# LuoGroup2023/PanTax

Hardware: AMD Instinct MI355X
Metric: PAO wall-time (s) + Mreads/s: packed reads + DB (graphs and their unique-trio index) resident in HBM -> abundance tables; the metric's own GAF -> abundance quantity is value_gaf_to_tables (files -> tables, never `value`) (higher is better)
Workload: dtype int64+f64

## Files before the change

pantax_amd/csrc/common.hpp:

```cpp
#pragma once
#include <hip/hip_runtime.h>
#include <cstdint>
#include <cstdio>
#include <map>
#include <functional>
#include <mutex>
#include <cstring>
#include <atomic>
#include <string>
#include <vector>
#include "../../include/pantax_hip.h"

#ifndef TRIO_LH_PACK
#define TRIO_LH_PACK 0
#endif
namespace ptx {

struct Ctx;
#if TRIO_LH_PACK
using trio_len_t = uint2;
#else
using trio_len_t = uint32_t;
#endif

// ... 274 lines not shown
    DevBuf<uint32_t> d_sp_first_id;
    DevBuf<uint32_t> d_node_base;
    DevBuf<uint64_t> d_bit_off;
    DevBuf<uint32_t> d_node_len;
    DevBuf<uint4> d_node_rec;
    DevBuf<uint64_t> d_path_off;
    DevBuf<uint32_t> d_path_nodes;
    DevBuf<uint32_t> d_hap_species;
    DevBuf<uint64_t> d_hap_off;
    DevBuf<uint8_t> d_all_same;
    std::vector<uint8_t> h_all_same;
    DevBuf<uint2> d_tiles;
    uint64_t n_tiles = 0;
    DevBuf<uint2> d_emit_tile_sp;
    DevBuf<uint64_t> d_node_haps;
    bool nh_built = false, nh_walk_too = false;
    DevBuf<uint32_t> d_tile_rank;
    DevBuf<uint32_t> d_hap_tile_off;
    bool trio_visit_ok = false;
    uint32_t n_vgroups = 0;
    std::vector<uint8_t> h_trio_slow;
    DevBuf<uint32_t> d_trio_slow;
    DevBuf<uint32_t> d_vis_pos;
    DevBuf<uint64_t> d_vis_head;
    DevBuf<uint32_t> d_vis_nbase;
    DevBuf<uint32_t> d_vis_sp;
    DevBuf<uint32_t> d_node_visited;
    bool trio_block_ok = false;
    uint32_t n_blocks = 0;
    uint64_t n_runs = 0;
    DevBuf<uint32_t> d_blk_base;
    DevBuf<uint32_t> d_blk_species;
    DevBuf<uint32_t> d_blk_run_off;
    DevBuf<uint4> d_blk_rec;
    DevBuf<uint4> d_runs;
    bool trio_built = false;
    bool trio_prefetched = false;
    bool trio_keys_built = false;
    bool trio_perm_valid = false;
    uint64_t U = 0;
    bool cov_prepared = false;
    bool cov_count_pending = false;
    bool cov_self_clean = false, cov_arena_clean = false;
    uint64_t cov_arena_sig = 0;
    size_t cov_arena_total = 0;
    hipEvent_t ev_cov_read = nullptr, ev_cov_clean = nullptr;
    bool cov_clean_pending = false;
    bool trio_sizes_known = false;
    uint64_t U_known = 0;
    bool trio_layout_fast = false;
    DevBuf<uint32_t> d_trio_first;
    DevBuf<uint2> d_trio_ent;
#if TRIO_LH_PACK
    DevBuf<uint2> d_trio_len;
#else
    DevBuf<uint32_t> d_trio_len;
    DevBuf<uint16_t> d_trio_hap;
#endif
    DevBuf<uint32_t> d_trio_q;
    DevBuf<uint32_t> d_trio_perm;
    DevBuf<uint64_t> d_hap_trio_off;
    std::vector<uint64_t> h_hap_trio_off;
    std::vector<uint32_t> h_sp_row_order;
    struct NodeChunks { DevBuf<uint32_t> d_chunk_sp, d_sp_off; uint32_t n = 0; };
    NodeChunks node_chunks[2];
    DevBuf<uint4> d_stat_chunks;
    DevBuf<double> d_hs_x;
    DevBuf<uint16_t> d_hs_h;
    DevBuf<uint32_t> d_hs_n;
    uint32_t n_stat_chunks = 0;
    uint64_t n_stat_partials = 0;
    uint32_t stat_lds_haps = 0;
    bool stat_global_rows = false;
    DevBuf<uint32_t> d_sp_chunk_off;
    bool cov_done = false;
    bool cov_stage = false;
    DevBuf<uint8_t> d_cov_arena;
    unsigned long long *d_abort = nullptr;
    DevBuf<unsigned long long> d_bases;
    DevBuf<uint32_t> d_bitmap;
    uint64_t item_sel_layout = 0;
    uint32_t item_sel_n = 0;
    bool item_sel_on = false;
    DevBuf<uint32_t> d_item_sel;
    DevBuf<uint32_t> d_full;
    DevBuf<uint32_t> d_cov;
    DevBuf<unsigned long long> d_trio_bases;
    DevBuf<uint8_t> d_active;
    DevBuf<uint8_t> d_ones;
    DevBuf<unsigned long long> d_counters;
    TrioScratch trio_scratch;
    LadBatch lad;
    DevBuf<uint32_t> d_hap_nnz;
    DevBuf<double> d_hap_mean;
    DevBuf<double> d_hap_part;
    DevBuf<uint8_t> d_arena;
    PinBuf h_arena[2];
    DevBuf<double> d_avg_len, d_sp_abs;
    DevBuf<uint8_t> d_sp_out;
    PinBuf h_sp_out[2];
    hipEvent_t ev_step[2] = {nullptr, nullptr};
    pantax_hip_step_config step_cfg[2];
    int stats_slot = -1;
    int step_enq = 0, step_col = 0, step_inflight = 0;
    hipEvent_t ev_trio_free = nullptr;
    bool trio_free_valid = false;
    bool trio_free_pending = false;
    ~Db() { for (hipEvent_t e : ev_step) if (e) (void)hipEventDestroy(e); if (ev_trio_free) (void)hipEventDestroy(ev_trio_free);
            if (ev_cov_read) (void)hipEventDestroy(ev_cov_read); if (ev_cov_clean) (void)hipEventDestroy(ev_cov_clean); }
    DevBuf<uint32_t> d_scan_tmp, d_sort_table, d_ss_ws;
    DevBuf<uint64_t> d_ka[3], d_kb[3];
    DevBuf<uint64_t> d_row16;
};

struct Reads {
    uint64_t R = 0, T = 0;
    DevBuf<uint32_t> d_step_off, d_node_id, d_pstart, d_pend, d_qlen;
    DevBuf<uint8_t> d_mapq, d_flags;
    DevBuf<uint64_t> d_id_hash;
    bool has_flags = false;
    DevBuf<int32_t> d_species;
    std::vector<int32_t> h_pre_species;
    std::vector<uint32_t> h_pre_qlen;
    uint64_t T_pad = 0;
    DevBuf<uint32_t> d_g_node_id, d_g_group_slot, d_slot_of;
    DevBuf<uint4> d_g_read_rec;
    DevBuf<uint8_t> d_g_step_dup;
    DevBuf<uint32_t> d_long_sum;
    DevBuf<uint32_t> d_long_len0;
    uint32_t n_long = 0;
    DevBuf<uint2> d_g_slot_rec;
    DevBuf<uint2> d_g_qm;
    DevBuf<uint2> d_g_mm;
    DevBuf<uint8_t> d_g_flag;
    uint32_t n_slots = 0;
    DevBuf<uint2> d_g_items;
    uint32_t n_items = 0;
    int item_blk_shift = 0;
    bool g_flags_valid = false;
    bool species_valid = false;
    bool binned = false;
    uint64_t binned_db = 0;
    bool grouped = true;
    uint64_t layout_id = 0;
    uint64_t long_sums_db = 0;
    std::vector<uint32_t> h_item_block;
    uint32_t max_node_id = 0;
};

__host__ __device__ inline int slot_species(int32_t x) { return x >= -1 ? x : -x - 2; }

constexpr uint64_t NODE_REC_MAX_BITS = 1ull << 40;
constexpr uint32_t NODE_REC_MAX_ROWS = 1u << 16;
__host__ __device__ inline uint32_t nr_rows(uint32_t y) { return (y >> 8) & 0xFFFFu; }
__host__ __device__ inline uint32_t nr_filter(uint32_t y) { return y >> 24; }
__host__ __device__ inline uint32_t nr_head(uint32_t y_old, uint32_t rows, uint32_t filter) { return (y_old & 0xFFu) | ((rows & 0xFFFFu) << 8) | (filter << 24); }
__host__ __device__ inline uint32_t nr_pair_bit(uint32_t lo, uint32_t hi) { return 1u << (((lo * 0x9E3779B1u) ^ (hi * 0x85EBCA77u)) >> 29); }
__host__ __device__ inline uint64_t nr_bit_off(const uint4 &r) { return ((uint64_t)(r.y & 0xFFu) << 32) | r.x; }
__host__ __device__ inline uint4 nr_make(uint64_t bit_off, uint32_t len) { return make_uint4((uint32_t)bit_off, (uint32_t)(bit_off >> 32) & 0xFFu, len, 0u); }

template <class T>
int upload(Ctx *ctx, DevBuf<T> &dst, const T *src, size_t n) {
    PTX_HIP(ctx, dst.alloc(n));
    if (n) PTX_HIP(ctx, hipMemcpyAsync(dst.p, src, n * sizeof(T), hipMemcpyHostToDevice, ctx->stream));
    return 0;
}
// ... 137 lines not shown
```

pantax_amd/csrc/cov_device.hpp:

```cpp
#pragma once
#include "common.hpp"
#include "wave.hpp"

namespace ptx {

constexpr int COV_BLOCK = 256;

__device__ __forceinline__ uint32_t bm_peek(const uint32_t *p) {
    return __hip_atomic_load(p, __ATOMIC_RELAXED, __HIP_MEMORY_SCOPE_AGENT);
}
constexpr uint32_t COV_BWIN = 2048;
constexpr int COV_WIN = 2048;
extern __shared__ uint32_t s_cov[];
#define S_WIN(i) s_cov[(i)]
#define S_BM(bmo, i) s_cov[(bmo) + (i)]
#define S_FULL(bmo, i) reinterpret_cast<uint8_t *>(s_cov + (bmo) + COV_BWIN)[(i)]
__host__ __device__ constexpr size_t cov_lds_bytes(int win) { return (size_t)win * 4 + COV_BWIN * 4 + (size_t)win; }
__device__ __forceinline__ void lds_or(uint32_t *__restrict__ bm, uint32_t bmo, uint64_t bw0, uint32_t bwn, uint64_t w, uint32_t m) {
    const uint64_t off = w - bw0;
    if (off < bwn) {
        if ((S_BM(bmo, off) & m) != m) atomicOr(&S_BM(bmo, off), m);
    } else if ((bm_peek(&bm[w]) & m) != m) atomicOr(&bm[w], m);
}
__device__ __forceinline__ void mark_range(uint32_t *__restrict__ bm, uint32_t bmo, uint64_t bw0, uint32_t bwn, uint64_t g0, uint64_t g1) {
    if (g1 <= g0) return;
    uint64_t w0 = g0 >> 5, w1 = (g1 - 1) >> 5;
    uint32_t m0 = 0xFFFFFFFFu << (g0 & 31);
    uint32_t m1 = 0xFFFFFFFFu >> (31 - (uint32_t)((g1 - 1) & 31));
    if (w0 == w1) lds_or(bm, bmo, bw0, bwn, w0, m0 & m1);
    else {
        lds_or(bm, bmo, bw0, bwn, w0, m0);
        for (uint64_t w = w0 + 1; w < w1; ++w) lds_or(bm, bmo, bw0, bwn, w, 0xFFFFFFFFu);
        lds_or(bm, bmo, bw0, bwn, w1, m1);
    }
}
__device__ __forceinline__ void win_or(uint32_t bmo, uint32_t w, uint32_t m) { if ((S_BM(bmo, w) & m) != m) atomicOr(&S_BM(bmo, w), m); }
__device__ __forceinline__ void mark_window(uint32_t bmo, uint32_t r0, uint32_t r1) {
    if (r1 <= r0) return;
    const uint32_t w0 = r0 >> 5, w1 = (r1 - 1) >> 5;
    const uint32_t m0 = 0xFFFFFFFFu << (r0 & 31), m1 = 0xFFFFFFFFu >> (31 - ((r1 - 1) & 31));
    if (w0 == w1) win_or(bmo, w0, m0 & m1);
    else {
        win_or(bmo, w0, m0);
        for (uint32_t w = w0 + 1; w < w1; ++w) win_or(bmo, w, 0xFFFFFFFFu);
        win_or(bmo, w1, m1);
    }
}

constexpr uint32_t STEP_LONG = 0x80u;
constexpr uint32_t STEP_START = 0x40u, STEP_PAD = 0xFFu, STEP_DIST = 0x3Fu;
__device__ __forceinline__ unsigned long long ballot1(bool b) { return __builtin_amdgcn_ballot_w64(b); }
__device__ __forceinline__ bool any1(bool b) { return __builtin_amdgcn_ballot_w64(b) != 0ull; }
__device__ __forceinline__ bool none1(bool b) { return __builtin_amdgcn_ballot_w64(b) == 0ull; }
__device__ __forceinline__ uint32_t slot_in_group(uint32_t group_first_slot, uint32_t code, int lane) {
    const unsigned long long starts = ballot1((code != STEP_PAD) & ((code & STEP_START) != 0u)) & ~1ull;
    const uint32_t below = __builtin_amdgcn_mbcnt_hi((uint32_t)(starts >> 32), __builtin_amdgcn_mbcnt_lo((uint32_t)starts, 0u));
    return group_first_slot + below + (uint32_t)((starts >> lane) & 1ull);
}

__device__ __forceinline__ uint32_t rl_from_memory(uint32_t j, uint32_t b, const uint32_t *__restrict__ node_id, const uint8_t *__restrict__ step_dup,
                                                   uint32_t delta, const uint4 *__restrict__ node_rec, uint32_t len0, uint32_t ps) {
    const uint32_t idj = node_id[b + j];
    if (j == 0 || ((step_dup[b + j] & 1u) && idj == node_id[b])) return len0 - ps;
    return node_rec[idj + delta].z;
}

#ifdef COV_ABLATE
#define ABL(bit) (ablate & (bit))
#else
#define ABL(bit) false
#endif
constexpr int COV_WIN_BACK = 128;
constexpr uint32_t NO_SLOT = 0xFFFFFFFFu;

__device__ __forceinline__ void add_bases(unsigned long long *__restrict__ bases, uint32_t wlo, uint32_t win_n, uint32_t v, uint32_t aln) {
    const uint32_t off = v - wlo;
    if (off < win_n && aln < (1u << 18)) atomicAdd(&S_WIN(off), aln);
    else atomicAdd(&bases[v], (unsigned long long)aln);
}
constexpr uint32_t NO_FULL = 0xFFFFFFFFu;
__device__ __forceinline__ void mark_full_wave(uint32_t *__restrict__ full, uint32_t wlo, uint32_t win_n, uint32_t v) {
    const uint32_t off = v - wlo;
    const bool have = v != NO_FULL;
    if (have && off < win_n) S_FULL(COV_WIN, off) = 1;
    const bool out = have && off >= win_n;
    unsigned long long todo = __ballot(out);
    const uint32_t w = v >> 5, bit = 1u << (v & 31);
    const int lane = threadIdx.x & 63;
    while (todo) {
        const int leader = __builtin_ctzll(todo);
        const uint32_t wl = (uint32_t)__builtin_amdgcn_readlane((int)w, leader);
        const bool mine = out && w == wl;
        const uint32_t orv = wave_reduce(mine ? bit : 0u, [](uint32_t x, uint32_t y) { return x | y; });
        if (lane == leader) atomicOr(&full[wl], orv);
        todo &= ~__ballot(mine);
    }
}

constexpr uint32_t COV_ITEM_GROUPS = 128;
struct __attribute__((packed, aligned(4))) EntPair { uint32_t a, b, c, d; };
constexpr int COV_BLK_SHIFT = 11;

template <int WIN>
__device__ __forceinline__ void mark_full_out_wave(uint32_t *__restrict__ full, bool out, uint32_t v) {
    unsigned long long todo = ballot1(out);
    const uint32_t w = v >> 5, bit = 1u << (v & 31);
    const int lane = threadIdx.x & 63;
    while (todo) {
        const int leader = __builtin_ctzll(todo);
        const uint32_t wl = (uint32_t)__builtin_amdgcn_readlane((int)w, leader);
        const bool mine = out & (w == wl);
        const uint32_t orv = wave_reduce(mine ? bit : 0u, [](uint32_t x, uint32_t y) { return x | y; });
        if (lane == leader) atomicOr(&full[wl], orv);
        todo &= ~ballot1(mine);
    }
}

}
```

pantax_amd/csrc/stage_cov.hip:

```cpp
#include <chrono>
#include <cstdio>
#include <cstdlib>
#include "common.hpp"
#include "primitives.hpp"
#include "wave.hpp"
#include "cov_plan.hpp"
#include "cov_device.hpp"
#pragma clang diagnostic ignored "-Wbitwise-instead-of-logical"

namespace ptx {

template <bool WITH_TRIO, int U, int PASSES, int WIN, bool LONG = false>
__global__ void __launch_bounds__(COV_BLOCK) coverage_fast_kernel(
    const uint2 *__restrict__ items, const uint32_t *__restrict__ group_slot, const uint4 *__restrict__ read_rec, const uint2 *__restrict__ slot_rec,
    const uint32_t *__restrict__ node_id, const uint8_t *__restrict__ step_code, const uint8_t *__restrict__ active,
    const uint4 *__restrict__ node_rec, const uint64_t *__restrict__ bit_off, uint64_t V, unsigned long long *__restrict__ bases,
    uint32_t *__restrict__ bitmap, uint32_t *__restrict__ full, const uint2 *__restrict__ trio_ent, unsigned long long *__restrict__ trio_bases,
    unsigned long long *__restrict__ n_abort, uint32_t ablate, int blk_shift,
    const uint32_t *__restrict__ long_sum = nullptr, const uint32_t *__restrict__ long_len0 = nullptr, uint32_t only_long = 0u,
    uint32_t chunk_groups = 0u, uint32_t total_groups = 0u, uint32_t win_back = 0u, const uint32_t *__restrict__ item_sel = nullptr) {
    constexpr int WAVES = COV_BLOCK / 64;
    const int lane = threadIdx.x & 63, wave = threadIdx.x >> 6;
    uint32_t g0, n_groups;
    if constexpr (LONG) { g0 = blockIdx.x * chunk_groups; n_groups = min(g0 + chunk_groups, total_groups); }
    else { const uint2 item = items[item_sel ? item_sel[blockIdx.x] : blockIdx.x]; g0 = item.x; n_groups = item.y; }
    for (int i = threadIdx.x; i < (int)(cov_lds_bytes(WIN) / 4); i += COV_BLOCK) s_cov[i] = 0;
    uint32_t wlo = 0, win_n = 0, mark_n = 0, bit0_lo = 0, bwn = 0;
    uint64_t bw0 = 0;
#pragma unroll 1
    for (uint32_t g = g0; g < n_groups && win_n == 0; ++g) {
        const uint32_t gs = group_slot[g];
        if (gs == NO_SLOT) continue;
        const uint2 sr0 = slot_rec[gs];
        if ((int)sr0.x < 0 || !active[sr0.x]) continue;
        const uint32_t id0 = node_id[(uint64_t)g * 64], v0 = id0 + sr0.y, in_blk = id0 & ((1u << blk_shift) - 1u);
        const uint32_t back = LONG ? win_back : in_blk + 64u;
        wlo = (v0 > back ? v0 - back : 0u) & ~63u;
        win_n = WIN;
        const uint64_t b_lo = bit_off[wlo], b_hi = bit_off[min((uint64_t)wlo + WIN, V)];
        bw0 = b_lo >> 5;
        bit0_lo = (uint32_t)(bw0 << 5);
        bwn = COV_BWIN;
        mark_n = (b_hi - (bw0 << 5) <= (uint64_t)COV_BWIN * 32) ? (uint32_t)min((uint64_t)WIN, V - wlo) : 0u;
    }
    __builtin_amdgcn_fence(__ATOMIC_RELEASE, "workgroup", "local");
    __builtin_amdgcn_s_barrier();
    __builtin_amdgcn_fence(__ATOMIC_ACQUIRE, "workgroup", "local");
#ifndef COV_NO_PREFETCH
    uint32_t n_code[U], n_id[U], n_gs[U];
    {
        const uint32_t gw0 = g0 + (uint32_t)(wave * U);
#pragma unroll
        for (int u = 0; u < U; ++u) {
            const uint32_t g = gw0 + (uint32_t)u < n_groups ? gw0 + (uint32_t)u : (gw0 < n_groups ? gw0 : g0);
            const uint64_t t = (uint64_t)g * 64 + lane;
            n_code[u] = step_code[t]; n_id[u] = node_id[t]; n_gs[u] = group_slot[g];
        }
    }
#endif
#if !defined(COV_NO_PF2) && !defined(COV_NO_PREFETCH)
    constexpr bool PF2 = !LONG;
#else
    constexpr bool PF2 = false;
#endif
    uint32_t c_code[U], c_id[U], c_gs[U];
    uint4 c_rr[U];
    uint2 c_sr[U];
    bool c_run[U];
#pragma unroll
    for (int u = 0; u < U; ++u) c_run[u] = false;
    if constexpr (PF2) {
        const uint32_t gw0 = g0 + (uint32_t)(wave * U), gw1 = gw0 + (uint32_t)(WAVES * U);
#pragma unroll
        for (int u = 0; u < U; ++u) {
            c_code[u] = n_code[u]; c_id[u] = n_id[u]; c_gs[u] = n_gs[u];
            const uint32_t g = gw1 + (uint32_t)u < n_groups ? gw1 + (uint32_t)u : (gw0 < n_groups ? gw0 : g0);
            const uint64_t t = (uint64_t)g * 64 + lane;
            n_code[u] = step_code[t]; n_id[u] = node_id[t]; n_gs[u] = group_slot[g];
            const bool pad0 = c_code[u] == STEP_PAD;
            const bool run0 = (gw0 + (uint32_t)u < n_groups) & any1(!pad0) & none1(!pad0 & ((c_code[u] & STEP_LONG) != 0u));
            const uint32_t sl = slot_in_group(c_gs[u], c_code[u], lane);
            const uint32_t slot = (pad0 | !run0) ? (c_gs[u] == NO_SLOT ? 0u : c_gs[u]) : sl;
            c_rr[u] = read_rec[slot]; c_sr[u] = slot_rec[slot];
            c_run[u] = run0;
        }
    }
#pragma unroll 1
    for (int pass = 0;; ++pass) {
        const uint32_t gw = g0 + (uint32_t)((pass * WAVES + wave) * U);
        if (gw >= n_groups) break;
        uint32_t code[U], id[U], gs[U];
        bool run[U];
        uint4 rr[U];
        uint2 sr[U];
#ifndef COV_NO_PREFETCH
        if constexpr (PF2) {
            const uint32_t gn = gw + (uint32_t)(WAVES * U), g2 = gn + (uint32_t)(WAVES * U);
            uint32_t m_code[U], m_id[U], m_gs[U];
#pragma unroll
            for (int u = 0; u < U; ++u) {
                run[u] = c_run[u];
                code[u] = c_code[u]; id[u] = c_id[u]; gs[u] = c_gs[u]; rr[u] = c_rr[u]; sr[u] = c_sr[u];
                const uint32_t g = g2 + (uint32_t)u < n_groups ? g2 + (uint32_t)u : gw;
                const uint64_t t = (uint64_t)g * 64 + lane;
                m_code[u] = step_code[t]; m_id[u] = node_id[t]; m_gs[u] = group_slot[g];
                const bool padn = n_code[u] == STEP_PAD;
                const bool runn = (gn + (uint32_t)u < n_groups) & any1(!padn) & none1(!padn & ((n_code[u] & STEP_LONG) != 0u));
                const uint32_t sl = slot_in_group(n_gs[u], n_code[u], lane);
                const uint32_t slot = (padn | !runn) ? (n_gs[u] == NO_SLOT ? 0u : n_gs[u]) : sl;
                c_rr[u] = read_rec[slot]; c_sr[u] = slot_rec[slot];
                c_run[u] = runn;
                c_code[u] = n_code[u]; c_id[u] = n_id[u]; c_gs[u] = n_gs[u];
                n_code[u] = m_code[u]; n_id[u] = m_id[u]; n_gs[u] = m_gs[u];
            }
        } else
        {
            const uint32_t gn = gw + (uint32_t)(WAVES * U);
#pragma unroll
            for (int u = 0; u < U; ++u) {
                run[u] = gw + (uint32_t)u < n_groups;
                code[u] = n_code[u]; id[u] = n_id[u]; gs[u] = n_gs[u];
                const uint32_t g = gn + (uint32_t)u < n_groups ? gn + (uint32_t)u : gw;
                const uint64_t t = (uint64_t)g * 64 + lane;
                n_code[u] = step_code[t]; n_id[u] = node_id[t]; n_gs[u] = group_slot[g];
            }
        }
#else
#pragma unroll
        for (int u = 0; u < U; ++u) {
            const uint32_t g = gw + (uint32_t)u;
            run[u] = g < n_groups;
            const uint64_t t = (uint64_t)(run[u] ? g : gw) * 64 + lane;
            code[u] = step_code[t]; id[u] = node_id[t];
            gs[u] = group_slot[run[u] ? g : gw];
        }
#endif
        bool pad[U];
        uint32_t ll0[U], lsum[U];
#pragma unroll
        for (int u = 0; u < U; ++u) {
            pad[u] = code[u] == STEP_PAD;
            if constexpr (!PF2) {
                const bool has_long = any1(!pad[u] & ((code[u] & STEP_LONG) != 0u));
                run[u] = run[u] & any1(!pad[u]) & (LONG ? (has_long | (only_long == 0u)) : !has_long);
            }
            const uint32_t sl = slot_in_group(gs[u], code[u], lane);
            const uint32_t slot = (pad[u] | !run[u]) ? (gs[u] == NO_SLOT ? 0u : gs[u]) : sl;
            if constexpr (!PF2) { rr[u] = read_rec[slot]; sr[u] = slot_rec[slot]; }
            if constexpr (LONG) { ll0[u] = long_len0[slot]; lsum[u] = long_sum[slot]; }
        }
        uint32_t h_id1[U], h_id2[U], h_codes[U];
        if constexpr (LONG) {
#pragma unroll
            for (int u = 0; u < U; ++u) {
                const uint32_t gu = (uint32_t)__builtin_amdgcn_readfirstlane((int)(gw + (uint32_t)u));
                const uint64_t t0 = (uint64_t)(run[u] && gu != 0u ? gu : 1u) * 64;
                h_id1[u] = node_id[t0 - 1]; h_id2[u] = node_id[t0 - 2];
                h_codes[u] = *reinterpret_cast<const uint32_t *>(step_code + t0 - 4);
            }
        }
        uint4 nr[U];
// ... 48 lines not shown
            dead_read[u] = !single[u] & (rr[u].z > len0[u]);
            live[u] = ok[u] & !dead_read[u] & !(single[u] & (rr[u].w < rr[u].z));
            nh[u] = 0; hx[u] = 0; tlo[u] = 0; thi[u] = 0;
            e0[u] = make_uint2(0u, 0u); e1[u] = e0[u];
            if (WITH_TRIO && !ABL(4u)) {
                hx[u] = hw1;
                tlo[u] = min(v[u], v2); thi[u] = max(v[u], v2);
                nh[u] = (live[u] & (i_[u] >= 2u) & ((nr_filter(hy1) & nr_pair_bit(tlo[u], thi[u])) != 0u)) ? nr_rows(hy1) : 0u;
                const EntPair ep = *reinterpret_cast<const EntPair *>(trio_ent + (nh[u] ? hx[u] : 0u));
                e0[u] = make_uint2(ep.a, ep.b); e1[u] = make_uint2(ep.c, ep.d);
            }
        }
#pragma unroll
        for (int u = 0; u < U; ++u) {
            const uint32_t k = rr[u].y, ps = rr[u].z, pe = rr[u].w, i = i_[u];
            if (any1(ok[u] & dead_read[u] & (i == 0u))) { if (ok[u] & dead_read[u] & (i == 0u)) atomicAdd(n_abort, 1ull); }
            const uint32_t contrib = (live[u] & !single[u]) ? (i == 0u ? nl[u] - ps : nl[u]) : 0u;
            const uint32_t pexcl = wave_incl_scan_dpp(contrib) - contrib;
            uint32_t seen = pexcl - __shfl(pexcl, lane - (LONG ? dist[u] : (int)i));
            if constexpr (LONG) seen = cross[u] ? lsum[u] - ps : seen;
            const uint32_t tgt = pe - ps;
            uint32_t aln = nl[u];
            if (i + 1u == k) aln = ((pe >= ps) & (tgt > seen)) ? tgt - seen : 0u;
            if (i == 0u) aln = single[u] ? tgt : nl[u] - ps;
            const uint32_t sidx = i == 0u ? ps : 0u;
            uint32_t hi = sidx + aln;
            if (hi > nl[u]) hi = nl[u];
            const bool markable = live[u] & (hi > sidx) & !(single[u] & !((ps < pe) & (pe <= nl[u])));
            const uint32_t dupd = code[u] & STEP_DIST;
            bool earlier = dupd != 0u, at_step0 = dupd == i;
            if constexpr (LONG) {
                const bool lc = (code[u] & STEP_LONG) != 0u;
                const uint32_t id_first = cross[u] ? idf[u] : __shfl(id[u], lane - dist[u]);
                earlier = lc ? (code[u] & 1u) != 0u : earlier;
                at_step0 = lc ? id[u] == id_first : at_step0;
            }
            const uint32_t rl = !live[u] ? 0u : !earlier ? aln : (at_step0 ? len0[u] - ps : nl[u]);
            const uint32_t off = v[u] - wlo;
            const bool inw = off < win_n;
            if (live[u] & !earlier & (aln != 0u) && !ABL(2u)) {
                if (inw & (aln < (1u << 18))) atomicAdd(&S_WIN(off), aln);
                else atomicAdd(&bases[v[u]], (unsigned long long)aln);
            }
            const bool whole = markable & (sidx == 0u) & (hi == nl[u]);
            if constexpr (LONG) { if (!ABL(1u) && !ABL(8u)) mark_full_out_wave<WIN>(full, whole & !inw, v[u]); }
            if (markable && !ABL(1u)) {
                if (whole) {
                    if (inw) S_FULL(WIN, off) = 1; else if (!LONG && !ABL(8u)) atomicOr(&full[v[u] >> 5], 1u << (v[u] & 31));
                } else if (off < mark_n) {
                    const uint32_t rel = nr[u].x - bit0_lo;
                    mark_window(WIN, rel + sidx, rel + hi);
                } else if (!ABL(8u)) {
                    const uint64_t bo = nr_bit_off(nr[u]);
                    mark_range(bitmap, WIN, bw0, bwn, bo + sidx, bo + hi);
                }
            }
            if (WITH_TRIO && !ABL(4u)) {
                uint32_t rl1 = wave_shr1(rl), rl2 = wave_shr1(rl1);
                if constexpr (LONG) {
                    const uint32_t idf0 = (uint32_t)__builtin_amdgcn_readfirstlane((int)idf[u]), l0 = (uint32_t)__builtin_amdgcn_readfirstlane((int)len0[u]),
                                   ps0 = (uint32_t)__builtin_amdgcn_readfirstlane((int)ps);
                    const uint32_t c1 = h_codes[u] >> 24, c2 = (h_codes[u] >> 16) & 0xFFu;
                    const uint32_t rlh1 = ((i0_[u] == 1u) | (((c1 & 1u) != 0u) & (h_id1[u] == idf0))) ? l0 - ps0 : nrh1[u].z;
                    const uint32_t rlh2 = ((i0_[u] == 2u) | (((c2 & 1u) != 0u) & (h_id2[u] == idf0))) ? l0 - ps0 : nrh2[u].z;
                    rl2 = lane == 0 ? rlh2 : lane == 1 ? rlh1 : rl2;
                    rl1 = lane == 0 ? rlh1 : rl1;
                }
                constexpr uint32_t NO_ROW = 0xFFFFFFFFu;
                const bool m0 = (nh[u] != 0u) & (e0[u].x == tlo[u]) & (e0[u].y == thi[u]);
                const bool m1 = (nh[u] > 1u) & (e1[u].x == tlo[u]) & (e1[u].y == thi[u]);
                uint32_t row = m0 ? hx[u] : m1 ? hx[u] + 1u : NO_ROW;
                if (any1(!(m0 | m1) & (nh[u] > 2u))) {
                    if (!(m0 | m1) & (nh[u] > 2u))
                        for (uint32_t j = 2; j < nh[u]; ++j) {
                            const uint2 e = trio_ent[hx[u] + j];
                            if (e.x == tlo[u] && e.y == thi[u]) { row = hx[u] + j; break; }
                        }
                }
                const uint32_t sum = rl2 + rl1 + rl;
                if ((row != NO_ROW) & (sum != 0u)) atomicAdd(&trio_bases[row], (unsigned long long)sum);
            }
        }
    }
    __syncthreads();
    if (win_n) {
        for (int i = threadIdx.x; i < WIN; i += COV_BLOCK) {
            const uint32_t c = S_WIN(i);
            if (c) atomicAdd(&bases[wlo + i], (unsigned long long)c);
            const unsigned long long fb = __ballot(S_FULL(WIN, i) != 0);
            if (fb && (lane & 31) == 0 && !ABL(32u)) {
                const uint32_t m = (uint32_t)(fb >> (lane & 32));
                if (m) atomicOr(&full[(wlo + i) >> 5], m);
            }
        }
        if (!ABL(16u))
        for (uint32_t i = threadIdx.x; i < bwn; i += COV_BLOCK) {
            const uint32_t m = S_BM(WIN, i);
            if (m) atomicOr(&bitmap[bw0 + i], m);
        }
    }
}

template <int WS_U, bool EAGER = false>
__global__ void __launch_bounds__(256) walk_sum_kernel(uint64_t T, const uint32_t *__restrict__ group_slot, const uint8_t *__restrict__ step_dup,
                                                       const uint4 *__restrict__ read_rec, const uint2 *__restrict__ slot_rec,
                                                       const uint32_t *__restrict__ node_id, const uint32_t *__restrict__ node_len,
                                                       uint32_t *__restrict__ long_sum, uint32_t *__restrict__ long_len0) {
    const int lane = threadIdx.x & 63;
    const uint64_t stride = (uint64_t)gridDim.x * 256 * WS_U;
    for (uint64_t base = ((uint64_t)blockIdx.x * 256 + (threadIdx.x - lane)) * WS_U; base < T; base += stride) {
        uint32_t code[WS_U], slot[WS_U], id[WS_U], nl[WS_U], gs_e[WS_U], id_e[WS_U];
        uint64_t t[WS_U];
        bool any = false;
#pragma unroll
        for (int u = 0; u < WS_U; ++u) {
            t[u] = base + (uint64_t)u * 64 + lane;
            code[u] = t[u] < T ? step_dup[t[u]] : STEP_PAD;
            if constexpr (EAGER) { gs_e[u] = t[u] < T ? group_slot[t[u] >> 6] : NO_SLOT; id_e[u] = t[u] < T ? node_id[t[u]] : 0u; }
        }
#pragma unroll
        for (int u = 0; u < WS_U; ++u) any = any || (code[u] != STEP_PAD && (code[u] & STEP_LONG));
        if (!__any(any)) continue;
#pragma unroll
        for (int u = 0; u < WS_U; ++u) {
            slot[u] = NO_SLOT; id[u] = 0;
            uint32_t gs;
            if constexpr (EAGER) gs = gs_e[u]; else gs = t[u] < T ? group_slot[t[u] >> 6] : NO_SLOT;
            const uint32_t sl = slot_in_group(gs, code[u], lane);
            if (code[u] != STEP_PAD && (code[u] & STEP_LONG)) { slot[u] = sl; if constexpr (EAGER) id[u] = id_e[u]; else id[u] = node_id[t[u]]; }
        }
        uint2 sr[WS_U];
        uint4 rr[WS_U];
#pragma unroll
        for (int u = 0; u < WS_U; ++u) {
            sr[u] = make_uint2(0xFFFFFFFFu, 0u); rr[u] = make_uint4(0u, 0u, 0u, 0u);
            if (slot[u] != NO_SLOT) { sr[u] = slot_rec[slot[u]]; rr[u] = read_rec[slot[u]]; }
        }
#pragma unroll
        for (int u = 0; u < WS_U; ++u) {
            nl[u] = 0;
            const bool counted = slot[u] != NO_SLOT && (int)sr[u].x >= 0 && (uint32_t)(t[u] - rr[u].x) + 1 < rr[u].y;
            if (counted) nl[u] = node_len[id[u] + sr[u].y];
        }
#pragma unroll
        for (int u = 0; u < WS_U; ++u) {
            if (!__any(slot[u] != NO_SLOT)) continue;
            if (slot[u] != NO_SLOT && (int)sr[u].x >= 0 && (uint32_t)(t[u] - rr[u].x) + 1 < rr[u].y && t[u] == rr[u].x)
                long_len0[slot[u]] = nl[u];
            const uint32_t prev = __shfl_up(slot[u], 1);
            const bool head = lane == 0 || prev != slot[u];
            const unsigned long long heads = __ballot(head);
            const int start = 63 - __builtin_clzll(heads & ((2ull << lane) - 1ull));
            const uint32_t sc = wave_incl_scan_dpp(nl[u]);
            const uint32_t front = __shfl(sc, start > 0 ? start - 1 : 0);
            const uint32_t incl = sc - (start > 0 ? front : 0u);
            const unsigned long long after = heads & ~((2ull << lane) - 1ull);
            const bool tail = after ? (lane + 1 == __builtin_ctzll(after)) : lane == 63;
            if (tail && slot[u] != NO_SLOT && incl) atomicAdd(&long_sum[slot[u]], incl);
        }
    }
}

__global__ void __launch_bounds__(256) popcount_kernel(uint64_t V, const uint64_t *__restrict__ bit_off, const uint32_t *__restrict__ full,
                                                       const uint32_t *__restrict__ bitmap, uint32_t *__restrict__ cov) {
    for (uint64_t v = (uint64_t)blockIdx.x * 256 + threadIdx.x; v < V; v += (uint64_t)gridDim.x * 256) {
        uint64_t g0 = bit_off[v], g1 = bit_off[v + 1];
        uint32_t c = 0;
        if ((full[v >> 5] >> (uint32_t)(v & 31)) & 1u) c = (uint32_t)(g1 - g0);
        else if (g1 > g0) {
            uint64_t w0 = g0 >> 5, w1 = (g1 - 1) >> 5;
            uint32_t m0 = 0xFFFFFFFFu << (g0 & 31);
            uint32_t m1 = 0xFFFFFFFFu >> (31 - (uint32_t)((g1 - 1) & 31));
            if (w0 == w1) c = __popc(bitmap[w0] & m0 & m1);
            else {
                c = __popc(bitmap[w0] & m0);
                for (uint64_t w = w0 + 1; w < w1; ++w) c += __popc(bitmap[w]);
                c += __popc(bitmap[w1] & m1);
            }
        }
        cov[v] = c;
    }
}

// ... 80 lines not shown
            PTX_HIP(ctx, hipStreamSynchronize(ctx->stream));
            if (nz) return fail(ctx, PANTAX_HIP_E_STATE, "coverage_prepare: %llu non-zero words in an arena its last readers should have left clean", nz);
        }
        PTX_HIP(ctx, hipMemsetAsync(db->d_abort, 0, 8, ctx->stream));
    } else {
        KTimer t(ctx, "zero_fill_kernel");
        PTX_TRY(zero_fill(ctx, base, total));
    }
    db->cov_arena_clean = false;
    db->cov_arena_sig = sig;
    if (rd->R && rd->T_pad && rd->n_long && rd->long_sums_db != 0 && rd->long_sums_db == db->uid) {
    } else if (rd->R && rd->T_pad && rd->n_long) {
        PTX_HIP(ctx, hipMemsetAsync(rd->d_long_sum.p, 0, rd->R * sizeof(uint32_t), ctx->stream));
        KTimer t(ctx, "walk_sum_kernel");
        const bool eager = (uint64_t)rd->n_long * 2 > rd->n_slots;
        hipLaunchKernelGGL((eager ? walk_sum_kernel<4, true> : walk_sum_kernel<4, false>), dim3(grid_for(rd->T_pad / 4 + 1, 256, ctx->n_cu * 16)), dim3(256), 0, ctx->stream, rd->T_pad, rd->d_g_group_slot.p,
                           rd->d_g_step_dup.p, rd->d_g_read_rec.p, rd->d_g_slot_rec.p, rd->d_g_node_id.p, db->d_node_len.p, rd->d_long_sum.p,
                           rd->d_long_len0.p);
    }
    PTX_HIP(ctx, hipGetLastError());
    db->cov_prepared = true;
    return 0;
}

int coverage_arena_clean_async(Ctx *ctx, Db *db) {
    if (!db->d_cov_arena.p || !db->cov_arena_total || !ctx->stream2) return 0;
    uint8_t *f_ptr = db->d_cov_arena.p;
    const size_t f_n = db->cov_arena_total;
    if (!db->ev_cov_read) PTX_HIP(ctx, hipEventCreateWithFlags(&db->ev_cov_read, hipEventDisableTiming));
    if (!db->ev_cov_clean) PTX_HIP(ctx, hipEventCreateWithFlags(&db->ev_cov_clean, hipEventDisableTiming));
    PTX_HIP(ctx, hipEventRecord(db->ev_cov_read, ctx->stream));
    PTX_HIP(ctx, hipStreamWaitEvent(ctx->stream2, db->ev_cov_read, 0));
    hipStream_t main_stream = ctx->stream;
    ctx->stream_main = main_stream; ctx->stream = ctx->stream2;
    int rc;
    rc = zero_fill(ctx, f_ptr, f_n);
    const hipError_t e = hipEventRecord(db->ev_cov_clean, ctx->stream2);
    ctx->stream = main_stream; ctx->stream_main = nullptr;
    if (rc != 0) return rc;
    PTX_HIP(ctx, e);
    db->cov_done = false;
    db->cov_arena_clean = true; db->cov_clean_pending = true;
    return 0;
}

struct CovLap {
    Ctx *ctx;
    bool on;
    std::chrono::steady_clock::time_point prev = std::chrono::steady_clock::now();
    void operator()(const char *what) {
        if (!on) return;
        (void)hipStreamSynchronize(ctx->stream);
        const auto now = std::chrono::steady_clock::now();
        std::fprintf(stderr, "[node_coverage]        %-28s %9.3f ms\n", what, std::chrono::duration<double, std::milli>(now - prev).count());
        prev = now;
    }
};

static int active_flags(Ctx *ctx, Db *db, const uint8_t *d_active, const uint8_t **out) {
    if (!d_active) {
        if (db->d_ones.n < db->S) { PTX_HIP(ctx, db->d_ones.alloc(db->S)); PTX_HIP(ctx, hipMemsetAsync(db->d_ones.p, 1, db->S, ctx->stream)); }
        d_active = db->d_ones.p;
    }
    *out = d_active;
    return 0;
}

struct ItemList { uint32_t n; const uint32_t *d; };
static int item_selection(Ctx *ctx, Db *db, const Reads *rd, ItemList *out) {
    *out = {rd->n_items, nullptr};
    if (db->item_sel_layout == rd->layout_id && rd->layout_id != 0) {
        *out = {db->item_sel_n, db->item_sel_on ? db->d_item_sel.p : nullptr};
    } else if (rd->h_item_block.size() == rd->n_items && rd->item_blk_shift > 0 && db->S && !db->h_range_start.empty()) {
        const CovItemSel s = cov_item_select(rd->h_item_block, rd->item_blk_shift, db->h_range_start, db->h_range_end);
        if (s.on && s.n_sel) PTX_TRY(upload(ctx, db->d_item_sel, s.sel.data(), s.sel.size()));
        *out = {s.n_sel, s.on && s.n_sel ? db->d_item_sel.p : nullptr};
        db->item_sel_layout = rd->layout_id; db->item_sel_n = s.n_sel; db->item_sel_on = s.on;
    }
    return 0;
}

struct CovFastTail {
    const uint2 *items; int blk_shift; const uint32_t *long_sum, *long_len0; uint32_t only_long, chunk_groups, total_groups, win_back; const uint32_t *item_sel;
};
template <int U, int PASSES, int WIN, bool LONG>
static void fast_launch_as(Ctx *ctx, Db *db, Reads *rd, const uint8_t *d_act, bool trio, int grid, const CovFastTail &t) {
    if (grid <= 0) return;
    const auto kernel = trio ? coverage_fast_kernel<true, U, PASSES, WIN, LONG> : coverage_fast_kernel<false, U, PASSES, WIN, LONG>;
    hipLaunchKernelGGL(kernel, dim3(grid), dim3(COV_BLOCK), cov_lds_bytes(WIN), ctx->stream, t.items, rd->d_g_group_slot.p, rd->d_g_read_rec.p,
                       rd->d_g_slot_rec.p, rd->d_g_node_id.p, rd->d_g_step_dup.p, d_act, db->d_node_rec.p, db->d_bit_off.p, db->V, db->d_bases.p,
                       db->d_bitmap.p, db->d_full.p, db->d_trio_ent.p, db->d_trio_bases.p, db->d_abort, ctx->cfg.cov_ablate ,
                       t.blk_shift, t.long_sum, t.long_len0, t.only_long, t.chunk_groups, t.total_groups, t.win_back, t.item_sel);
}

static int fast_launch(Ctx *ctx, Db *db, Reads *rd, const uint8_t *d_act, bool trio, const CovFastShape &f, const ItemList &list) {
    const CovFastTail t{rd->d_g_items.p, rd->item_blk_shift, nullptr, nullptr, 0u, 0u, 0u, 0u, list.d};
    const int grid = (int)list.n;
    const auto is = [&](int u, int passes, int win) { return f.u == u && f.passes == passes && f.win == win; };
    if (is(1, 8, 2048)) fast_launch_as<1, 8, 2048, false>(ctx, db, rd, d_act, trio, grid, t);
    else if (is(2, 4, 2048)) fast_launch_as<2, 4, 2048, false>(ctx, db, rd, d_act, trio, grid, t);
    else if (is(2, 8, 2048)) fast_launch_as<2, 8, 2048, false>(ctx, db, rd, d_act, trio, grid, t);
    else if (is(2, 8, 3072)) fast_launch_as<2, 8, 3072, false>(ctx, db, rd, d_act, trio, grid, t);
    else if (is(2, 8, 4096)) fast_launch_as<2, 8, 4096, false>(ctx, db, rd, d_act, trio, grid, t);
    else if (is(2, 4, 3072)) fast_launch_as<2, 4, 3072, false>(ctx, db, rd, d_act, trio, grid, t);
    else if (is(2, 8, 2304)) fast_launch_as<2, 8, 2304, false>(ctx, db, rd, d_act, trio, grid, t);
    else if (is(2, 8, 2560)) fast_launch_as<2, 8, 2560, false>(ctx, db, rd, d_act, trio, grid, t);
    else if (is(2, 4, 2304)) fast_launch_as<2, 4, 2304, false>(ctx, db, rd, d_act, trio, grid, t);
    else if (is(2, 4, 2560)) fast_launch_as<2, 4, 2560, false>(ctx, db, rd, d_act, trio, grid, t);
    else if (is(1, 8, 2304)) fast_launch_as<1, 8, 2304, false>(ctx, db, rd, d_act, trio, grid, t);
    else if (is(4, 4, 2304)) fast_launch_as<4, 4, 2304, false>(ctx, db, rd, d_act, trio, grid, t);
    else if (is(4, 4, 2048)) fast_launch_as<4, 4, 2048, false>(ctx, db, rd, d_act, trio, grid, t);
    else if (is(4, 4, 3072)) fast_launch_as<4, 4, 3072, false>(ctx, db, rd, d_act, trio, grid, t);
    else return fail(ctx, PANTAX_HIP_E_STATE, "coverage_launch: no short-read kernel of shape U = %d, PASSES = %d, WIN = %d", f.u, f.passes, f.win);
    return 0;
}

static int long_launch(Ctx *ctx, Db *db, Reads *rd, const uint8_t *d_act, bool trio, const CovPlan &plan) {
    if (!rd->d_long_sum.p) { PTX_HIP(ctx, rd->d_long_sum.alloc(rd->R)); PTX_HIP(ctx, rd->d_long_len0.alloc(rd->R)); }
    const CovLongShape &l = plan.lng;
    const uint32_t total_groups = (uint32_t)(rd->T_pad / 64);
    const int grid = (int)((total_groups + l.chunk_groups - 1) / l.chunk_groups);
    const CovFastTail t{nullptr, 0, rd->d_long_sum.p, rd->d_long_len0.p, plan.only_long ? 1u : 0u, l.chunk_groups, total_groups, l.win_back, nullptr};
    if (l.u == 1 && l.win == 2048) fast_launch_as<1, 1, 2048, true>(ctx, db, rd, d_act, trio, grid, t);
    else if (l.u == 1 && l.win == 3072) fast_launch_as<1, 1, 3072, true>(ctx, db, rd, d_act, trio, grid, t);
    else if (l.u == 1 && l.win == 4096) fast_launch_as<1, 1, 4096, true>(ctx, db, rd, d_act, trio, grid, t);
    else if (l.u == 2 && l.win == 2048) fast_launch_as<2, 1, 2048, true>(ctx, db, rd, d_act, trio, grid, t);
    else if (l.u == 2 && l.win == 4096) fast_launch_as<2, 1, 4096, true>(ctx, db, rd, d_act, trio, grid, t);
    else if (l.u == 2 && l.win == 3072) fast_launch_as<2, 1, 3072, true>(ctx, db, rd, d_act, trio, grid, t);
    else return fail(ctx, PANTAX_HIP_E_STATE, "coverage_launch: no long-walk kernel of shape U = %d, WIN = %d", l.u, l.win);
    return 0;
}

static int count_launch(Ctx *ctx, Db *db) {
    PTX_HIP(ctx, db->d_cov.alloc(db->V));
    KTimer t(ctx, "popcount_kernel");
    if (long_node_shape(db->L, db->V, ctx->cfg.ncs_prefix_min, ctx->cfg.ncs_no_prefix))
        hipLaunchKernelGGL(popcount_long_kernel, dim3(grid_for((db->V + 63) / 64, 4, ctx->n_cu * 8)), dim3(256), 0, ctx->stream, db->V,
                           db->d_bit_off.p, db->d_full.p, db->d_bitmap.p, db->d_cov.p);
    else
        hipLaunchKernelGGL(popcount_kernel, dim3(grid_for(db->V, 256, ctx->n_cu * 8)), dim3(256), 0, ctx->stream, db->V,
                           db->d_bit_off.p, db->d_full.p, db->d_bitmap.p, db->d_cov.p);
    return 0;
}

int coverage_launch(Ctx *ctx, Db *db, Reads *rd, const uint8_t *d_active, bool with_trio, bool defer_count) {
    if (!rd->grouped) return fail(ctx, PANTAX_HIP_E_STATE, "node_coverage: these reads are a slice kept as plain columns (to be routed to their owner), not resident reads");
    const bool trace = ctx->cfg.trace && !defer_count;
    CovLap lap{ctx, trace};
    if (!db->cov_prepared) PTX_TRY(coverage_prepare(ctx, db, rd, with_trio));
    lap("arena + zero fill");
    db->cov_prepared = false;
    db->cov_stage = false;
    db->trio_free_valid = false;
    const bool trio = with_trio && db->U;
    const uint8_t *d_act_fast = d_active;
    if (rd->R && rd->T_pad) PTX_TRY(active_flags(ctx, db, d_active, &d_act_fast));
    const CtxConfig &cfg = ctx->cfg;
    const CovPlan plan = cov_plan(rd->T_pad, rd->n_long, rd->n_slots, rd->n_items, rd->R, cfg.cov_general, cfg.cov_long, cfg.covf_shape, cfg.covl_shape,
                                  cfg.cov_shape, cfg.cov_xcd);
    if (plan.run_fast) {
        KTimer t(ctx, "coverage_fast_kernel");
        ItemList list;
        PTX_TRY(item_selection(ctx, db, rd, &list));
        if (trace) std::fprintf(stderr, "[node_coverage]        %u of %u items launched\n", list.n, rd->n_items);
        PTX_TRY(fast_launch(ctx, db, rd, d_act_fast, trio, plan.fast, list));
    }
    if (plan.run_long) {
        KTimer t(ctx, "coverage_long_kernel");
        PTX_TRY(long_launch(ctx, db, rd, d_act_fast, trio, plan));
    }
    if (plan.run_step) {
        KTimer t(ctx, "coverage_step_kernel");
        PTX_TRY(coverage_step_launch(ctx, db, rd, d_active, trio, plan));
    }
    PTX_HIP(ctx, hipGetLastError());
    lap("coverage kernels");
    db->cov_count_pending = defer_count && db->V != 0;
    if (db->V && !defer_count) PTX_TRY(count_launch(ctx, db));
    PTX_HIP(ctx, hipGetLastError());
    lap("popcount");
    db->cov_done = true;
    return 0;
}

}
```

Measured before the change: 6851.

## Precompute per-item coverage windows in a separate kernel before the fast coverage pass

A new small kernel computes each selected item's window base, mark count and bitmap word offset ahead of time and stores them in a per-item buffer. The fast (non-long) coverage kernel then reads one uint4 per block instead of scanning its groups serially for the first active one. It also issues its step-code and node-id prefetch loads before zeroing LDS and hitting the barrier, so that latency overlaps with the setup. The cost is one extra launch and buffer, plus global traffic for the window records.

Result: no change. 6908, median of 2 (+0.8%).

```diff
diff --git a/pantax_amd/csrc/common.hpp b/pantax_amd/csrc/common.hpp
--- a/pantax_amd/csrc/common.hpp
+++ b/pantax_amd/csrc/common.hpp
@@ -380,6 +380,7 @@
     uint64_t item_sel_layout = 0;
     uint32_t item_sel_n = 0;
     bool item_sel_on = false;
+    DevBuf<uint4> d_item_win;
     DevBuf<uint32_t> d_item_sel;
     DevBuf<uint32_t> d_full;
     DevBuf<uint32_t> d_cov;
diff --git a/pantax_amd/csrc/cov_device.hpp b/pantax_amd/csrc/cov_device.hpp
--- a/pantax_amd/csrc/cov_device.hpp
+++ b/pantax_amd/csrc/cov_device.hpp
@@ -101,6 +101,32 @@
 struct __attribute__((packed, aligned(4))) EntPair { uint32_t a, b, c, d; };
 constexpr int COV_BLK_SHIFT = 11;
 
+constexpr uint32_t COV_WIN_DEAD = 0xFFFFFFFFu;
+__device__ __forceinline__ uint4 cov_item_window(uint32_t g0, uint32_t n_groups, const uint32_t *__restrict__ group_slot, const uint2 *__restrict__ slot_rec,
+                                                 const uint8_t *__restrict__ active, const uint32_t *__restrict__ node_id, const uint64_t *__restrict__ bit_off,
+                                                 uint64_t V, int blk_shift, uint32_t win, bool untested) {
+#pragma unroll 1
+    for (uint32_t g = g0; g < n_groups; ++g) {
+        uint32_t delta = 0;
+        if (!untested) {
+            const uint32_t gs = group_slot[g];
+            if (gs == NO_SLOT) continue;
+            const uint2 sr0 = slot_rec[gs];
+            if ((int)sr0.x < 0 || !active[sr0.x]) continue;
+            delta = sr0.y;
+        }
+        const uint32_t id0 = node_id[(uint64_t)g * 64], in_blk = id0 & ((1u << blk_shift) - 1u), back = in_blk + 64u;
+        uint32_t v0 = id0 + delta;
+        if (untested) v0 = (uint32_t)min((uint64_t)v0, V ? V - 1 : 0);
+        const uint32_t wlo = (v0 > back ? v0 - back : 0u) & ~63u;
+        const uint64_t b_lo = bit_off[wlo], b_hi = bit_off[min((uint64_t)wlo + win, V)];
+        const uint64_t bw0 = b_lo >> 5;
+        const uint32_t mark_n = (b_hi - (bw0 << 5) <= (uint64_t)COV_BWIN * 32) ? (uint32_t)min((uint64_t)win, V - wlo) : 0u;
+        return make_uint4(wlo, mark_n, (uint32_t)bw0, (uint32_t)(bw0 >> 32));
+    }
+    return make_uint4(0u, COV_WIN_DEAD, 0u, 0u);
+}
+
 template <int WIN>
 __device__ __forceinline__ void mark_full_out_wave(uint32_t *__restrict__ full, bool out, uint32_t v) {
     unsigned long long todo = ballot1(out);
diff --git a/pantax_amd/csrc/stage_cov.hip b/pantax_amd/csrc/stage_cov.hip
--- a/pantax_amd/csrc/stage_cov.hip
+++ b/pantax_amd/csrc/stage_cov.hip
@@ -18,65 +18,89 @@
     uint32_t *__restrict__ bitmap, uint32_t *__restrict__ full, const uint2 *__restrict__ trio_ent, unsigned long long *__restrict__ trio_bases,
     unsigned long long *__restrict__ n_abort, uint32_t ablate, int blk_shift,
     const uint32_t *__restrict__ long_sum = nullptr, const uint32_t *__restrict__ long_len0 = nullptr, uint32_t only_long = 0u,
-    uint32_t chunk_groups = 0u, uint32_t total_groups = 0u, uint32_t win_back = 0u, const uint32_t *__restrict__ item_sel = nullptr) {
+    uint32_t chunk_groups = 0u, uint32_t total_groups = 0u, uint32_t win_back = 0u, const uint32_t *__restrict__ item_sel = nullptr,
+    const uint4 *__restrict__ item_win = nullptr) {
     constexpr int WAVES = COV_BLOCK / 64;
-    const int lane = threadIdx.x & 63, wave = threadIdx.x >> 6;
+    const int lane = threadIdx.x & 63, wave = LONG ? (int)(threadIdx.x >> 6) : __builtin_amdgcn_readfirstlane((int)(threadIdx.x >> 6));
     uint32_t g0, n_groups;
-    if constexpr (LONG) { g0 = blockIdx.x * chunk_groups; n_groups = min(g0 + chunk_groups, total_groups); }
-    else { const uint2 item = items[item_sel ? item_sel[blockIdx.x] : blockIdx.x]; g0 = item.x; n_groups = item.y; }
-    for (int i = threadIdx.x; i < (int)(cov_lds_bytes(WIN) / 4); i += COV_BLOCK) s_cov[i] = 0;
     uint32_t wlo = 0, win_n = 0, mark_n = 0, bit0_lo = 0, bwn = 0;
     uint64_t bw0 = 0;
+    uint4 wrec = make_uint4(0u, COV_WIN_DEAD, 0u, 0u);
+    if constexpr (LONG) {
+        g0 = blockIdx.x * chunk_groups; n_groups = min(g0 + chunk_groups, total_groups);
+        for (int i = threadIdx.x; i < (int)(cov_lds_bytes(WIN) / 4); i += COV_BLOCK) s_cov[i] = 0;
 #pragma unroll 1
-    for (uint32_t g = g0; g < n_groups && win_n == 0; ++g) {
-        const uint32_t gs = group_slot[g];
-        if (gs == NO_SLOT) continue;
-        const uint2 sr0 = slot_rec[gs];
-        if ((int)sr0.x < 0 || !active[sr0.x]) continue;
-        const uint32_t id0 = node_id[(uint64_t)g * 64], v0 = id0 + sr0.y, in_blk = id0 & ((1u << blk_shift) - 1u);
-        const uint32_t back = LONG ? win_back : in_blk + 64u;
-        wlo = (v0 > back ? v0 - back : 0u) & ~63u;
-        win_n = WIN;
-        const uint64_t b_lo = bit_off[wlo], b_hi = bit_off[min((uint64_t)wlo + WIN, V)];
-        bw0 = b_lo >> 5;
-        bit0_lo = (uint32_t)(bw0 << 5);
-        bwn = COV_BWIN;
-        mark_n = (b_hi - (bw0 << 5) <= (uint64_t)COV_BWIN * 32) ? (uint32_t)min((uint64_t)WIN, V - wlo) : 0u;
-    }
-    __builtin_amdgcn_fence(__ATOMIC_RELEASE, "workgroup", "local");
-    __builtin_amdgcn_s_barrier();
-    __builtin_amdgcn_fence(__ATOMIC_ACQUIRE, "workgroup", "local");
-#ifndef COV_NO_PREFETCH
-    uint32_t n_code[U], n_id[U], n_gs[U];
-    {
-        const uint32_t gw0 = g0 + (uint32_t)(wave * U);
-#pragma unroll
-        for (int u = 0; u < U; ++u) {
-            const uint32_t g = gw0 + (uint32_t)u < n_groups ? gw0 + (uint32_t)u : (gw0 < n_groups ? gw0 : g0);
-            const uint64_t t = (uint64_t)g * 64 + lane;
-            n_code[u] = step_code[t]; n_id[u] = node_id[t]; n_gs[u] = group_slot[g];
-        }
-    }
-#endif
+        for (uint32_t g = g0; g < n_groups && win_n == 0; ++g) {
+            const uint32_t gs = group_slot[g];
+            if (gs == NO_SLOT) continue;
+            const uint2 sr0 = slot_rec[gs];
+            if ((int)sr0.x < 0 || !active[sr0.x]) continue;
+            const uint32_t id0 = node_id[(uint64_t)g * 64], v0 = id0 + sr0.y;
+            wlo = (v0 > win_back ? v0 - win_back : 0u) & ~63u;
+            win_n = WIN;
+            const uint64_t b_lo = bit_off[wlo], b_hi = bit_off[min((uint64_t)wlo + WIN, V)];
+            bw0 = b_lo >> 5;
+            bit0_lo = (uint32_t)(bw0 << 5);
+            bwn = COV_BWIN;
+            mark_n = (b_hi - (bw0 << 5) <= (uint64_t)COV_BWIN * 32) ? (uint32_t)min((uint64_t)WIN, V - wlo) : 0u;
+        }
+        __builtin_amdgcn_fence(__ATOMIC_RELEASE, "workgroup", "local");
+        __builtin_amdgcn_s_barrier();
+        __builtin_amdgcn_fence(__ATOMIC_ACQUIRE, "workgroup", "local");
+    } else {
+        const uint2 item = items[item_sel ? item_sel[blockIdx.x] : blockIdx.x];
+        wrec = item_win[blockIdx.x];
+        g0 = item.x; n_groups = item.y;
+    }
 #if !defined(COV_NO_PF2) && !defined(COV_NO_PREFETCH)
     constexpr bool PF2 = !LONG;
 #else
     constexpr bool PF2 = false;
 #endif
+    uint32_t n_code[U], n_id[U], n_gs[U];
     uint32_t c_code[U], c_id[U], c_gs[U];
     uint4 c_rr[U];
     uint2 c_sr[U];
     bool c_run[U];
+    {
+#ifndef COV_NO_PREFETCH
+        const uint32_t gw0 = g0 + (uint32_t)(wave * U), gw1 = gw0 + (uint32_t)(WAVES * U);
+#pragma unroll
+        for (int u = 0; u < U; ++u) {
+            const uint32_t g = gw0 + (uint32_t)u < n_groups ? gw0 + (uint32_t)u : (gw0 < n_groups ? gw0 : g0);
+            const uint64_t t = (uint64_t)g * 64 + lane;
+            if constexpr (PF2) { c_code[u] = step_code[t]; c_id[u] = node_id[t]; c_gs[u] = group_slot[g]; }
+            else { n_code[u] = step_code[t]; n_id[u] = node_id[t]; n_gs[u] = group_slot[g]; }
+        }
+        if constexpr (PF2) {
+#pragma unroll
+            for (int u = 0; u < U; ++u) {
+                const uint32_t g = gw1 + (uint32_t)u < n_groups ? gw1 + (uint32_t)u : (gw0 < n_groups ? gw0 : g0);
+                const uint64_t t = (uint64_t)g * 64 + lane;
+                n_code[u] = step_code[t]; n_id[u] = node_id[t]; n_gs[u] = group_slot[g];
+            }
+        }
+#endif
+    }
+    if constexpr (!LONG) {
+        for (int i = threadIdx.x; i < (int)(cov_lds_bytes(WIN) / 4); i += COV_BLOCK) s_cov[i] = 0;
+        __builtin_amdgcn_fence(__ATOMIC_RELEASE, "workgroup", "local");
+        __builtin_amdgcn_s_barrier();
+        __builtin_amdgcn_fence(__ATOMIC_ACQUIRE, "workgroup", "local");
+#ifdef COV_ABLATE
+        if (ABL(256u)) wrec = cov_item_window(g0, n_groups, group_slot, slot_rec, active, node_id, bit_off, V, blk_shift, (uint32_t)WIN, ABL(64u) != 0u);
+#endif
+        const bool has = wrec.y != COV_WIN_DEAD;
+        wlo = wrec.x; win_n = has ? (uint32_t)WIN : 0u; mark_n = has ? wrec.y : 0u;
+        bw0 = (uint64_t)wrec.z | ((uint64_t)wrec.w << 32);
+        bit0_lo = (uint32_t)(bw0 << 5); bwn = has ? COV_BWIN : 0u;
+    }
 #pragma unroll
     for (int u = 0; u < U; ++u) c_run[u] = false;
     if constexpr (PF2) {
-        const uint32_t gw0 = g0 + (uint32_t)(wave * U), gw1 = gw0 + (uint32_t)(WAVES * U);
+        const uint32_t gw0 = g0 + (uint32_t)(wave * U);
 #pragma unroll
         for (int u = 0; u < U; ++u) {
-            c_code[u] = n_code[u]; c_id[u] = n_id[u]; c_gs[u] = n_gs[u];
-            const uint32_t g = gw1 + (uint32_t)u < n_groups ? gw1 + (uint32_t)u : (gw0 < n_groups ? gw0 : g0);
-            const uint64_t t = (uint64_t)g * 64 + lane;
-            n_code[u] = step_code[t]; n_id[u] = node_id[t]; n_gs[u] = group_slot[g];
             const bool pad0 = c_code[u] == STEP_PAD;
             const bool run0 = (gw0 + (uint32_t)u < n_groups) & any1(!pad0) & none1(!pad0 & ((c_code[u] & STEP_LONG) != 0u));
             const uint32_t sl = slot_in_group(c_gs[u], c_code[u], lane);
@@ -291,8 +315,13 @@
             }
         }
     }
-    __syncthreads();
-    if (win_n) {
+    if constexpr (LONG) __syncthreads();
+    else {
+        __builtin_amdgcn_fence(__ATOMIC_RELEASE, "workgroup", "local");
+        __builtin_amdgcn_s_barrier();
+        __builtin_amdgcn_fence(__ATOMIC_ACQUIRE, "workgroup", "local");
+    }
+    if (win_n && !ABL(128u)) {
         for (int i = threadIdx.x; i < WIN; i += COV_BLOCK) {
             const uint32_t c = S_WIN(i);
             if (c) atomicAdd(&bases[wlo + i], (unsigned long long)c);
@@ -308,6 +337,17 @@
             if (m) atomicOr(&bitmap[bw0 + i], m);
         }
     }
+}
+
+__global__ void __launch_bounds__(256) cov_item_window_kernel(uint32_t n, const uint2 *__restrict__ items, const uint32_t *__restrict__ item_sel,
+                                                              const uint32_t *__restrict__ group_slot, const uint2 *__restrict__ slot_rec,
+                                                              const uint8_t *__restrict__ active, const uint32_t *__restrict__ node_id,
+                                                              const uint64_t *__restrict__ bit_off, uint64_t V, int blk_shift, uint32_t win,
+                                                              uint4 *__restrict__ item_win) {
+    const uint32_t i = blockIdx.x * 256u + threadIdx.x;
+    if (i >= n) return;
+    const uint2 item = items[item_sel ? item_sel[i] : i];
+    item_win[i] = cov_item_window(item.x, item.y, group_slot, slot_rec, active, node_id, bit_off, V, blk_shift, win, false);
 }
 
 template <int WS_U, bool EAGER = false>
@@ -554,6 +594,7 @@
 
 struct CovFastTail {
     const uint2 *items; int blk_shift; const uint32_t *long_sum, *long_len0; uint32_t only_long, chunk_groups, total_groups, win_back; const uint32_t *item_sel;
+    const uint4 *item_win;
 };
 template <int U, int PASSES, int WIN, bool LONG>
 static void fast_launch_as(Ctx *ctx, Db *db, Reads *rd, const uint8_t *d_act, bool trio, int grid, const CovFastTail &t) {
@@ -562,11 +603,11 @@
     hipLaunchKernelGGL(kernel, dim3(grid), dim3(COV_BLOCK), cov_lds_bytes(WIN), ctx->stream, t.items, rd->d_g_group_slot.p, rd->d_g_read_rec.p,
                        rd->d_g_slot_rec.p, rd->d_g_node_id.p, rd->d_g_step_dup.p, d_act, db->d_node_rec.p, db->d_bit_off.p, db->V, db->d_bases.p,
                        db->d_bitmap.p, db->d_full.p, db->d_trio_ent.p, db->d_trio_bases.p, db->d_abort, ctx->cfg.cov_ablate ,
-                       t.blk_shift, t.long_sum, t.long_len0, t.only_long, t.chunk_groups, t.total_groups, t.win_back, t.item_sel);
+                       t.blk_shift, t.long_sum, t.long_len0, t.only_long, t.chunk_groups, t.total_groups, t.win_back, t.item_sel, t.item_win);
 }
 
 static int fast_launch(Ctx *ctx, Db *db, Reads *rd, const uint8_t *d_act, bool trio, const CovFastShape &f, const ItemList &list) {
-    const CovFastTail t{rd->d_g_items.p, rd->item_blk_shift, nullptr, nullptr, 0u, 0u, 0u, 0u, list.d};
+    const CovFastTail t{rd->d_g_items.p, rd->item_blk_shift, nullptr, nullptr, 0u, 0u, 0u, 0u, list.d, db->d_item_win.p};
     const int grid = (int)list.n;
     const auto is = [&](int u, int passes, int win) { return f.u == u && f.passes == passes && f.win == win; };
     if (is(1, 8, 2048)) fast_launch_as<1, 8, 2048, false>(ctx, db, rd, d_act, trio, grid, t);
@@ -587,12 +628,21 @@
     return 0;
 }
 
+static int item_window_launch(Ctx *ctx, Db *db, Reads *rd, const uint8_t *d_act, const ItemList &list, int win) {
+    if (!list.n) return 0;
+    PTX_HIP(ctx, db->d_item_win.alloc(list.n));
+    KTimer t(ctx, "cov_item_window_kernel");
+    hipLaunchKernelGGL(cov_item_window_kernel, dim3((list.n + 255) / 256), dim3(256), 0, ctx->stream, list.n, rd->d_g_items.p, list.d, rd->d_g_group_slot.p,
+                       rd->d_g_slot_rec.p, d_act, rd->d_g_node_id.p, db->d_bit_off.p, db->V, rd->item_blk_shift, (uint32_t)win, db->d_item_win.p);
+    return 0;
+}
+
 static int long_launch(Ctx *ctx, Db *db, Reads *rd, const uint8_t *d_act, bool trio, const CovPlan &plan) {
     if (!rd->d_long_sum.p) { PTX_HIP(ctx, rd->d_long_sum.alloc(rd->R)); PTX_HIP(ctx, rd->d_long_len0.alloc(rd->R)); }
     const CovLongShape &l = plan.lng;
     const uint32_t total_groups = (uint32_t)(rd->T_pad / 64);
     const int grid = (int)((total_groups + l.chunk_groups - 1) / l.chunk_groups);
-    const CovFastTail t{nullptr, 0, rd->d_long_sum.p, rd->d_long_len0.p, plan.only_long ? 1u : 0u, l.chunk_groups, total_groups, l.win_back, nullptr};
+    const CovFastTail t{nullptr, 0, rd->d_long_sum.p, rd->d_long_len0.p, plan.only_long ? 1u : 0u, l.chunk_groups, total_groups, l.win_back, nullptr, nullptr};
     if (l.u == 1 && l.win == 2048) fast_launch_as<1, 1, 2048, true>(ctx, db, rd, d_act, trio, grid, t);
     else if (l.u == 1 && l.win == 3072) fast_launch_as<1, 1, 3072, true>(ctx, db, rd, d_act, trio, grid, t);
     else if (l.u == 1 && l.win == 4096) fast_launch_as<1, 1, 4096, true>(ctx, db, rd, d_act, trio, grid, t);
@@ -631,10 +681,11 @@
     const CovPlan plan = cov_plan(rd->T_pad, rd->n_long, rd->n_slots, rd->n_items, rd->R, cfg.cov_general, cfg.cov_long, cfg.covf_shape, cfg.covl_shape,
                                   cfg.cov_shape, cfg.cov_xcd);
     if (plan.run_fast) {
-        KTimer t(ctx, "coverage_fast_kernel");
         ItemList list;
         PTX_TRY(item_selection(ctx, db, rd, &list));
         if (trace) std::fprintf(stderr, "[node_coverage]        %u of %u items launched\n", list.n, rd->n_items);
+        PTX_TRY(item_window_launch(ctx, db, rd, d_act_fast, list, plan.fast.win));
+        KTimer t(ctx, "coverage_fast_kernel");
         PTX_TRY(fast_launch(ctx, db, rd, d_act_fast, trio, plan.fast, list));
     }
     if (plan.run_long) {
```
